# twice154/ofa-for-super-resolution

Hardware: AMD Instinct MI355X
Metric: sr_training_images_per_sec_4x_64to256 (higher is better)
Workload: dtype bf16; 1 GPU; OFA-SR S4 supernet 4x progressive shrinking (elastic kernel {3,5,7}, e=6, d=4, pd=2), LR 64x64 -> HR 256x256, fwd+bwd+Adam, train-mode BN; kernel_transform_mode=1, compat_reference_indexing=True, parallelism=dp1, per_gpu_batch=16, global_batch=16, grad_allreduce_bytes=0, launch=eager

## Files before the change

ofa-for-super-resolution_amd/csrc/pwconv.hip:

```cpp
#include <stdlib.h>
#include "ofasr_common.h"

namespace ofasr {

typedef __attribute__((ext_vector_type(16))) float f32x16;
typedef __attribute__((ext_vector_type(8))) __bf16 bf16x8;
typedef __attribute__((ext_vector_type(8))) _Float16 f16x8;
typedef __attribute__((ext_vector_type(4))) short s16x4;
typedef __attribute__((ext_vector_type(8))) short s16x8;
typedef __attribute__((address_space(3))) s16x4 lds_s16x4;

constexpr int PW_THREADS = 256;
constexpr int PW_TILE = 128;
constexpr int XROW16 = 320;
constexpr int XROW32 = 512;
constexpr int WROW16 = 128;
constexpr int WROW32 = 256;

template <typename T> struct Mma16;
template <> struct Mma16<bf16_t> {
    static __device__ __forceinline__ f32x16 run(s16x8 a, s16x8 b, f32x16 c) {
        return __builtin_amdgcn_mfma_f32_32x32x16_bf16(__builtin_bit_cast(bf16x8, a), __builtin_bit_cast(bf16x8, b),
                                                       c, 0, 0, 0);
    }
// ... 1177 lines not shown

template <typename T> struct Rows64 {
    static constexpr int NIT = Elem<T>::is16 ? 2 : 4;
    static constexpr int CPR = Elem<T>::is16 ? 8 : 16;
    static constexpr int EPC = Elem<T>::is16 ? 8 : 4;
    uint4 v[NIT];
    uint32_t ok;
};
template <typename T>
__device__ __forceinline__ void rows64_request(Rows64<T>& g, const T* __restrict__ base, int rows_total, int r0, int HW, int p0) {
    const int tid = threadIdx.x;
    g.ok = 0;
#pragma unroll
    for (int it = 0; it < Rows64<T>::NIT; ++it) {
        const int q = tid + it * PW_THREADS;
        const int r = q / Rows64<T>::CPR, ch = q % Rows64<T>::CPR;
        const int px = p0 + Rows64<T>::EPC * ch;
        const bool ok = r0 + r < rows_total && px < HW;
        g.v[it] = *reinterpret_cast<const uint4*>(base + (ok ? (long long)(r0 + r) * HW + px : 0));
        g.ok |= (ok ? 1u : 0u) << it;
    }
}
template <typename T>
__device__ __forceinline__ void rows64_deposit(char* Lt, const Rows64<T>& g) {
    const int tid = threadIdx.x;
#pragma unroll
    for (int it = 0; it < Rows64<T>::NIT; ++it) {
        const int q = tid + it * PW_THREADS;
        const int r = q / Rows64<T>::CPR, ch = q % Rows64<T>::CPR;
        const uint32_t m = (g.ok >> it) & 1u ? 0xffffffffu : 0u;
        *reinterpret_cast<uint4*>(Lt + wtile_chunk_off<T>(r, ch)) = make_uint4(g.v[it].x & m, g.v[it].y & m, g.v[it].z & m, g.v[it].w & m);
    }
}

template <typename T, bool ALIGNED>
__global__ void __launch_bounds__(PW_THREADS) pw_wgrad_kernel(const T* __restrict__ R, const T* __restrict__ S,
                                                              float* __restrict__ part, int MR, int NS, int HW,
                                                              int stages_per_img, int total_stages,
                                                              int stages_per_split) {
    constexpr int SUB = WgStage<T>::SUB;
    constexpr int TB = 64 * Elem<T>::wrow;
    __shared__ __attribute__((aligned(16))) char Rt[SUB * TB];
    __shared__ __attribute__((aligned(16))) char St[SUB * TB];
    const int r0 = blockIdx.x * 64, s0 = blockIdx.y * 64, z = blockIdx.z;
    const int lane = lane_id();
    const int wave = __builtin_amdgcn_readfirstlane((int)(threadIdx.x >> 6));
    const int c = lane & 31, h = lane >> 5;
    const int rb = wave & 1, sb = wave >> 1;
    f32x16 acc = zero16();
    const int q_lo = z * stages_per_split;
    const int q_hi = min(total_stages, q_lo + stages_per_split);
    auto multiply = [&]() {
#pragma unroll
        for (int sub = 0; sub < SUB; ++sub) {
            const char* Rs = Rt + sub * TB;
            const char* Ss = St + sub * TB;
            if constexpr (Elem<T>::is16) {
#pragma unroll
                for (int s = 0; s < 4; ++s) {
                    const s16x8 af = *reinterpret_cast<const s16x8*>(Rs + wtile_chunk_off<T>(32 * rb + c, 2 * s + h));
                    const s16x8 bf = *reinterpret_cast<const s16x8*>(Ss + wtile_chunk_off<T>(32 * sb + c, 2 * s + h));
                    acc = Mma16<T>::run(af, bf, acc);
                }
            } else {
#pragma unroll
                for (int s4 = 0; s4 < 8; ++s4) {
                    const float4 a4 = *reinterpret_cast<const float4*>(Rs + wtile_chunk_off<T>(32 * rb + c, 8 * h + s4));
                    const float4 b4 = *reinterpret_cast<const float4*>(Ss + wtile_chunk_off<T>(32 * sb + c, 8 * h + s4));
                    acc = __builtin_amdgcn_mfma_f32_32x32x2f32(a4.x, b4.x, acc, 0, 0, 0);
                    acc = __builtin_amdgcn_mfma_f32_32x32x2f32(a4.y, b4.y, acc, 0, 0, 0);
                    acc = __builtin_amdgcn_mfma_f32_32x32x2f32(a4.z, b4.z, acc, 0, 0, 0);
                    acc = __builtin_amdgcn_mfma_f32_32x32x2f32(a4.w, b4.w, acc, 0, 0, 0);
                }
            }
        }
    };
    if constexpr (ALIGNED) {
        Rows64<T> rg[SUB], sg[SUB];
        auto request = [&](int q) {
            const int n = q / stages_per_img;
            const int p0 = (q - n * stages_per_img) * (64 * SUB);
#pragma unroll
            for (int sub = 0; sub < SUB; ++sub) {
                rows64_request<T>(rg[sub], R + (long long)n * MR * HW, MR, r0, HW, p0 + 64 * sub);
                rows64_request<T>(sg[sub], S + (long long)n * NS * HW, NS, s0, HW, p0 + 64 * sub);
            }
        };
        if (q_lo < q_hi) request(q_lo);
        for (int q = q_lo; q < q_hi; ++q) {
            if (q > q_lo) __syncthreads();
#pragma unroll
            for (int sub = 0; sub < SUB; ++sub) {
                rows64_deposit<T>(Rt + sub * TB, rg[sub]);
                rows64_deposit<T>(St + sub * TB, sg[sub]);
            }
            __syncthreads();
            if (q + 1 < q_hi) request(q + 1);
            multiply();
        }
    } else {
        for (int q = q_lo; q < q_hi; ++q) {
            const int n = q / stages_per_img;
            const int p0 = (q - n * stages_per_img) * (64 * SUB);
            if (q > q_lo) __syncthreads();
#pragma unroll
            for (int sub = 0; sub < SUB; ++sub) {
                stage_rows64<T, ALIGNED>(Rt + sub * TB, R + (long long)n * MR * HW, MR, r0, HW, p0 + 64 * sub);
                stage_rows64<T, ALIGNED>(St + sub * TB, S + (long long)n * NS * HW, NS, s0, HW, p0 + 64 * sub);
            }
            __syncthreads();
            multiply();
        }
    }
    float* pz = part + (long long)z * MR * NS;
    const int sc = s0 + 32 * sb + c;
#pragma unroll
    for (int reg = 0; reg < 16; ++reg) {
        const int rr = r0 + 32 * rb + acc_row(reg, h);
        if (rr < MR && sc < NS) pz[(long long)rr * NS + sc] = acc[reg];
    }
}

constexpr int WR_ZL = 16;
__global__ void __launch_bounds__(64 * WR_ZL) pw_wgrad_reduce_kernel(const float* __restrict__ part,
                                                                     float* __restrict__ dw, int MR, int NS, int nsplit,
                                                                     long long sr, long long ss) {
    __shared__ float red[WR_ZL][64];
    const long long tot = (long long)MR * NS;
    const long long idx = (long long)blockIdx.x * 64 + (threadIdx.x & 63);
    const int zl = threadIdx.x >> 6;
    float a = 0.f;
    if (idx < tot) {
        int z = zl;
        for (; z + 3 * WR_ZL < nsplit; z += 4 * WR_ZL) {
            const float v0 = part[(long long)z * tot + idx], v1 = part[(long long)(z + WR_ZL) * tot + idx];
            const float v2 = part[(long long)(z + 2 * WR_ZL) * tot + idx], v3 = part[(long long)(z + 3 * WR_ZL) * tot + idx];
            a += (v0 + v1) + (v2 + v3);
        }
        for (; z < nsplit; z += WR_ZL) a += part[(long long)z * tot + idx];
    }
    red[zl][threadIdx.x & 63] = a;
    __syncthreads();
    if (zl == 0 && idx < tot) {
        float t = 0.f;
#pragma unroll
        for (int i = 0; i < WR_ZL; ++i) t += red[i][threadIdx.x];
        const long long r = idx / NS, sx = idx - r * NS;
        dw[r * sr + sx * ss] = t;
    }
}

constexpr int WD_RB = 3;
constexpr int WD_ROWS = 4 * WD_RB * 32, WD_COLS = 64;

struct WdPlan {
    int quads_per_img, total_quads, nsplit, MR, NS;
};

template <typename T, int XF = 0>
__global__ void __launch_bounds__(512) pw_wgrad_direct_kernel(const T* __restrict__ R, const T* __restrict__ S,
                                                              float* __restrict__ part, int MR, int NS, int HW,
                                                              WdPlan wp, InputXf xf = InputXf{}, BwdXf bx = BwdXf{}) {
    const int lane = lane_id();
    const int wave = __builtin_amdgcn_readfirstlane((int)(threadIdx.x >> 6));
    const int wr = wave & 3, wc = wave >> 2;
    const int c = lane & 31, h = lane >> 5;
    const int split = blockIdx.x;
    const int row0 = blockIdx.y * WD_ROWS + wr * (WD_RB * 32);
    const int col = blockIdx.z * WD_COLS + wc * 32 + c;
    if (row0 >= MR) return;
    f32x16 acc[WD_RB];
#pragma unroll
    for (int rb = 0; rb < WD_RB; ++rb) acc[rb] = zero16();
    const int q0 = (int)((long long)split * wp.total_quads / wp.nsplit);
    const int q1 = (int)((long long)(split + 1) * wp.total_quads / wp.nsplit);
    const bool cs = col < NS;
    const int colc = cs ? col : NS - 1;
    bool rs[WD_RB];
    int rowc[WD_RB];
#pragma unroll
    for (int rb = 0; rb < WD_RB; ++rb) {
        rs[rb] = row0 + 32 * rb + c < MR;
        rowc[rb] = rs[rb] ? row0 + 32 * rb + c : MR - 1;
    }
    float xsc[WD_RB], xmu[WD_RB], xb[WD_RB];
    float csc = 1.f, cmu = 0.f, cbb = 0.f;
    if constexpr (XF == 1) {
#pragma unroll
        for (int rb = 0; rb < WD_RB; ++rb) {
            xsc[rb] = xf.scale[rowc[rb]];
            xmu[rb] = xf.mean[rowc[rb]];
            xb[rb] = fmaf(xmu[rb], xsc[rb], xf.shift[rowc[rb]]);
        }
    }
    if constexpr (XF == 2) {
        csc = xf.scale[colc];
        cmu = xf.mean[colc];
        cbb = fmaf(cmu, csc, xf.shift[colc]);
    }
    float bka[WD_RB], bkbi[WD_RB];
    if constexpr (XF == 3) {
#pragma unroll
        for (int rb = 0; rb < WD_RB; ++rb) {
            xsc[rb] = bx.scale[rowc[rb]];
            xmu[rb] = bx.mean[rowc[rb]];
            xb[rb] = fmaf(xmu[rb], xsc[rb], bx.shift[rowc[rb]]);
            bka[rb] = bx.ka[rowc[rb]];
            bkbi[rb] = bx.kbi[rowc[rb]];
        }
    }
    long long rowoff[WD_RB];
#pragma unroll
    for (int rb = 0; rb < WD_RB; ++rb) rowoff[rb] = (long long)rowc[rb] * HW;
    const long long coloff = (long long)colc * HW;
    for (int q = q0; q < q1; ++q) {
        const int n = q / wp.quads_per_img;
        const int px = (q - n * wp.quads_per_img) * 64 + 32 * h;
        uint4 a[WD_RB][4], b[4];
        bool okp[4];
        int pxc[4];
#pragma unroll
        for (int j = 0; j < 4; ++j) {
            okp[j] = px + 8 * j < HW;
            pxc[j] = okp[j] ? px + 8 * j : 0;
        }
        const T* sp = S + (long long)n * NS * HW + coloff;
#pragma unroll
        for (int j = 0; j < 4; ++j) b[j] = *reinterpret_cast<const uint4*>(sp + pxc[j]);
        const T* rn = R + (long long)n * MR * HW;
#pragma unroll
        for (int rb = 0; rb < WD_RB; ++rb) {
#pragma unroll
            for (int j = 0; j < 4; ++j) {
                a[rb][j] = *reinterpret_cast<const uint4*>(rn + rowoff[rb] + pxc[j]);
            }
        }
        uint4 ya[XF == 3 ? WD_RB : 1][4];
        if constexpr (XF == 3) {
            const T* yn = reinterpret_cast<const T*>(bx.y) + (long long)n * MR * HW;
#pragma unroll
            for (int rb = 0; rb < WD_RB; ++rb) {
#pragma unroll
                for (int j = 0; j < 4; ++j)
                    ya[rb][j] = *reinterpret_cast<const uint4*>(yn + rowoff[rb] + pxc[j]);
            }
        }
#pragma unroll
        for (int j = 0; j < 4; ++j) {
            if constexpr (XF == 2) b[j] = xf_apply8_core<T>(b[j], csc, cmu, cbb);
            if (!(cs && okp[j])) b[j] = make_uint4(0, 0, 0, 0);
        }
#pragma unroll
        for (int rb = 0; rb < WD_RB; ++rb)
#pragma unroll
            for (int j = 0; j < 4; ++j) {
                if constexpr (XF == 1) a[rb][j] = xf_apply8_core<T>(a[rb][j], xsc[rb], xmu[rb], xb[rb]);
                if constexpr (XF == 3) a[rb][j] = bx_apply8<T>(a[rb][j], ya[rb][j], xmu[rb], xsc[rb], xb[rb], bka[rb], bkbi[rb]);
                if (!(rs[rb] && okp[j])) a[rb][j] = make_uint4(0, 0, 0, 0);
            }
#pragma unroll
        for (int j = 0; j < 4; ++j)
#pragma unroll
            for (int rb = 0; rb < WD_RB; ++rb)
                acc[rb] = Mma16<T>::run(__builtin_bit_cast(s16x8, a[rb][j]), __builtin_bit_cast(s16x8, b[j]), acc[rb]);
    }
    float* dst = part + (long long)split * MR * NS;
    if (cs) {
        float* p = dst + (long long)(row0 + 4 * h) * NS + col;
#pragma unroll
        for (int rb = 0; rb < WD_RB; ++rb)
#pragma unroll
            for (int reg = 0; reg < 16; ++reg) {
                const int r = row0 + 32 * rb + acc_row(reg, h);
                if (r < MR) *p = acc[rb][reg];
                p += (reg & 3) == 3 ? 5 * (long long)NS : (long long)NS;
            }
    }
}

static WdPlan wd_plan(int64_t N, int64_t Cin, int64_t Cout, int64_t HW) {
    WdPlan p;
    p.MR = (int)(Cout >= Cin ? Cout : Cin);
    p.NS = (int)(Cout >= Cin ? Cin : Cout);
    p.quads_per_img = (int)cdiv(HW, 64);
    p.total_quads = (int)(N * p.quads_per_img);
    const int64_t tiles = cdiv(p.MR, WD_ROWS) * cdiv(p.NS, WD_COLS);
    static const int blocks = [] { const char* e = getenv("OFASR_PW_WGRAD_BLOCKS"); const int v = e ? atoi(e) : 0; return v > 0 ? v : 256; }();
    int64_t want = blocks / (tiles > 0 ? tiles : 1);
    if (want > p.total_quads / 4) want = p.total_quads / 4;
    if (want < 1) want = 1;
    p.nsplit = (int)want;
    return p;
}


struct WdPlan32 {
    int units_per_img, total_units, nsplit, MR, NS;
};

__global__ void __launch_bounds__(512) pw_wgrad_direct_f32_kernel(const float* __restrict__ R, const float* __restrict__ S,
                                                                  float* __restrict__ part, int MR, int NS, int HW,
                                                                  WdPlan32 wp) {
    const int lane = lane_id();
    const int wave = __builtin_amdgcn_readfirstlane((int)(threadIdx.x >> 6));
    const int wr = wave & 3, wc = wave >> 2;
    const int c = lane & 31, h = lane >> 5;
    const int split = blockIdx.x;
    const int row0 = blockIdx.y * WD_ROWS + wr * (WD_RB * 32);
    const int col = blockIdx.z * WD_COLS + wc * 32 + c;
    if (row0 >= MR) return;
    f32x16 acc[WD_RB];
#pragma unroll
    for (int rb = 0; rb < WD_RB; ++rb) acc[rb] = zero16();
    const int u0 = (int)((long long)split * wp.total_units / wp.nsplit);
    const int u1 = (int)((long long)(split + 1) * wp.total_units / wp.nsplit);
    const bool cs = col < NS;
    const int colc = cs ? col : NS - 1;
    bool rs[WD_RB];
    long long rowoff[WD_RB];
#pragma unroll
    for (int rb = 0; rb < WD_RB; ++rb) {
        rs[rb] = row0 + 32 * rb + c < MR;
        rowoff[rb] = (long long)(rs[rb] ? row0 + 32 * rb + c : MR - 1) * HW;
    }
    float4 a[2][WD_RB][4], b[2][4];
    auto request = [&](int set, int u) {
        const int uc = u < u1 ? u : u1 - 1;
        const int n = uc / wp.units_per_img;
        const int px = (uc - n * wp.units_per_img) * 32 + 16 * h;
        int pxc[4];
#pragma unroll
        for (int j = 0; j < 4; ++j) pxc[j] = px + 4 * j < HW ? px + 4 * j : 0;
        const float* sp = S + ((long long)n * NS + colc) * HW;
        const float* rp = R + (long long)n * MR * HW;
#pragma unroll
        for (int j = 0; j < 4; ++j) b[set][j] = *reinterpret_cast<const float4*>(sp + pxc[j]);
#pragma unroll
        for (int rb = 0; rb < WD_RB; ++rb)
#pragma unroll
            for (int j = 0; j < 4; ++j) a[set][rb][j] = *reinterpret_cast<const float4*>(rp + rowoff[rb] + pxc[j]);
    };
    auto multiply = [&](int set, int u) {
        const int n = u / wp.units_per_img;
        const int px = (u - n * wp.units_per_img) * 32 + 16 * h;
        const bool live = u < u1;
#pragma unroll
        for (int j = 0; j < 4; ++j) {
            const bool ok = live && cs && px + 4 * j < HW;
            const float4 bv = ok ? b[set][j] : make_float4(0.f, 0.f, 0.f, 0.f);
#pragma unroll
            for (int rb = 0; rb < WD_RB; ++rb) {
                const float4 av = rs[rb] ? a[set][rb][j] : make_float4(0.f, 0.f, 0.f, 0.f);
                acc[rb] = __builtin_amdgcn_mfma_f32_32x32x2f32(av.x, bv.x, acc[rb], 0, 0, 0);
                acc[rb] = __builtin_amdgcn_mfma_f32_32x32x2f32(av.y, bv.y, acc[rb], 0, 0, 0);
                acc[rb] = __builtin_amdgcn_mfma_f32_32x32x2f32(av.z, bv.z, acc[rb], 0, 0, 0);
                acc[rb] = __builtin_amdgcn_mfma_f32_32x32x2f32(av.w, bv.w, acc[rb], 0, 0, 0);
            }
        }
    };
    if (u0 < u1) {
        request(0, u0);
        for (int u = u0; u < u1; u += 2) {
            request(1, u + 1);
            multiply(0, u);
            request(0, u + 2);
            multiply(1, u + 1);
        }
    }
    float* dst = part + (long long)split * MR * NS;
    if (cs) {
        float* p = dst + (long long)(row0 + 4 * h) * NS + col;
#pragma unroll
        for (int rb = 0; rb < WD_RB; ++rb)
#pragma unroll
            for (int reg = 0; reg < 16; ++reg) {
                const int r = row0 + 32 * rb + acc_row(reg, h);
                if (r < MR) *p = acc[rb][reg];
                p += (reg & 3) == 3 ? 5 * (long long)NS : (long long)NS;
            }
    }
}

static WdPlan32 wd_plan32(int64_t N, int64_t Cin, int64_t Cout, int64_t HW) {
    WdPlan32 p;
    p.MR = (int)(Cout >= Cin ? Cout : Cin);
    p.NS = (int)(Cout >= Cin ? Cin : Cout);
    p.units_per_img = (int)cdiv(HW, 32);
    p.total_units = (int)(N * p.units_per_img);
    const int64_t tiles = cdiv(p.MR, WD_ROWS) * cdiv(p.NS, WD_COLS);
    int64_t want = 256 / (tiles > 0 ? tiles : 1);
    if (want > p.total_units / 8) want = p.total_units / 8;
    if (want < 1) want = 1;
    p.nsplit = (int)want;
    return p;
}

struct WgradPlan {
    int stages_per_img, total_stages, nsplit, stages_per_split, MR, NS;
};

static WgradPlan wgrad_plan(int64_t N, int64_t Cin, int64_t Cout, int64_t HW, int sub) {
    WgradPlan p;
    p.MR = (int)(Cout >= Cin ? Cout : Cin);
    p.NS = (int)(Cout >= Cin ? Cin : Cout);
    p.stages_per_img = (int)cdiv(HW, 64 * sub);
    p.total_stages = (int)(N * p.stages_per_img);
    const int64_t tiles = cdiv(p.MR, 64) * cdiv(p.NS, 64);
    int64_t want = 512 / (tiles > 0 ? tiles : 1);
    if (want < 1) want = 1;
    if (want > p.total_stages) want = p.total_stages;
    if (want < 1) want = 1;
    p.stages_per_split = (int)cdiv(p.total_stages, want);
    if (p.stages_per_split < 1) p.stages_per_split = 1;
    p.nsplit = (int)cdiv(p.total_stages, p.stages_per_split);
    if (p.nsplit < 1) p.nsplit = 1;
    return p;
}

static bool aligned_for(const void* a, const void* b, int64_t HW, bool is16) {
    const uintptr_t bits = reinterpret_cast<uintptr_t>(a) | reinterpret_cast<uintptr_t>(b);
    return (bits & 15) == 0 && (HW % (is16 ? 8 : 4)) == 0;
}

template <typename T, bool AL, bool WV, bool XF = false>
static void launch_gemm_v(const void* x, WView wv, void* y, int64_t HW, int tiles_per_img, int total_tiles,
                          hipStream_t st, InputXf xf = InputXf{}, const void* addend = nullptr,
                          StatOut so = StatOut{nullptr, 0}, BnFold fold = BnFold{}) {
    if (wv.K <= 64) {
        if constexpr (Elem<T>::is16 && AL && WV && !XF) {
            static const bool slabs = [] { const char* e = getenv("OFASR_PW_FANOUT_SLABS"); return !(e && e[0] == '0'); }();
            const int nslab = wv.M / FO_ROWS;
            if (slabs && addend == nullptr && wv.K == 64 && wv.M % FO_ROWS == 0 && (nslab == 2 || nslab == 3) &&
                HW % PW_TILE == 0) {
                dim3 g1((unsigned)total_tiles);
#define OFASR_FO_SLABS(NS, ST)                                                                                       \
    OFASR_LAUNCH((pw_fanout_slabs_kernel<T, NS, ST>), g1, dim3(PW_THREADS), 0, st, (const T*)x, wv, (T*)y, (int)HW, \
                       tiles_per_img, so, BwdStatOut{})
                if (nslab == 3) { if (so.partial) OFASR_FO_SLABS(3, 1); else OFASR_FO_SLABS(3, 0); }
                else { if (so.partial) OFASR_FO_SLABS(2, 1); else OFASR_FO_SLABS(2, 0); }
#undef OFASR_FO_SLABS
                return;
            }
        }
        dim3 grid((unsigned)total_tiles, (unsigned)cdiv(wv.M, FO_ROWS));
        OFASR_LAUNCH((pw_fanout_kernel<T, AL, WV, XF>), grid, dim3(PW_THREADS), 0, st, (const T*)x, wv, (T*)y,
                           (int)HW, tiles_per_img, xf, (const T*)addend, so);
    } else {
        dim3 grid((unsigned)total_tiles, (unsigned)cdiv(wv.M, 64));
        if constexpr (Elem<T>::is16 && AL && WV) {
            static const bool fast_ok = [] { const char* e = getenv("OFASR_PW_FANIN_FAST"); return !(e && e[0] == '0'); }();
            const bool span32 = (long long)wv.K * HW < (1LL << 31) &&
                                (long long)wv.M * wv.sm + (long long)wv.K * wv.sk < (1LL << 31);
            if (fast_ok && wv.K % 4 == 0 && wv.M % 4 == 0 && span32)
                OFASR_LAUNCH((pw_fanin_pipe_kernel<T, XF, true>), grid, dim3(PW_THREADS), 0, st, (const T*)x, wv,
                                   (T*)y, (int)HW, tiles_per_img, (int)cdiv(wv.K, 64), xf, (const T*)addend, so, fold);
            else
                OFASR_LAUNCH((pw_fanin_pipe_kernel<T, XF, false>), grid, dim3(PW_THREADS), 0, st, (const T*)x, wv,
                                   (T*)y, (int)HW, tiles_per_img, (int)cdiv(wv.K, 64), xf, (const T*)addend, so, fold);
            return;
        }
        OFASR_LAUNCH((pw_fanin_kernel<T, AL, WV, XF>), grid, dim3(PW_THREADS), 0, st, (const T*)x, wv, (T*)y,
                           (int)HW, tiles_per_img, (int)cdiv(wv.K, 64), xf, (const T*)addend, so);
    }
}

template <typename T, bool XF = false>
static int launch_gemm(const char* name, const void* x, WView wv, void* y, int64_t N, int64_t HW, hipStream_t st,
                       InputXf xf = InputXf{}, const void* addend = nullptr, StatOut so = StatOut{nullptr, 0},
                       BnFold fold = BnFold{}) {
    constexpr bool is16 = Elem<T>::is16;
    const bool al = aligned_for(x, y, HW, is16);
    const long long ld = wv.sk == 1 ? wv.sm : wv.sk;
    const bool wvec = (reinterpret_cast<uintptr_t>(wv.w) & 15) == 0 && (ld % 4) == 0 && wv.K % 4 == 0 && wv.M % 4 == 0;
    const int tiles_per_img = (int)cdiv(HW, PW_TILE);
    const int64_t total64 = N * tiles_per_img;
    OFASR_REQUIRE(total64 <= INT32_MAX, OFASR_ERR_UNSUPPORTED, "%s: too many pixel tiles", name);
    const int total_tiles = (int)total64;
    {
        const double px = (double)N * (double)HW, es = (double)sizeof(T);
        prof_note(es * px * (wv.K + wv.M + (addend ? wv.M : 0)) + 4.0 * wv.K * wv.M, 2.0 * px * wv.K * wv.M);
    }
    if (so.partial)
        OFASR_REQUIRE(so.P == (wv.K <= 64 ? total_tiles : 2 * total_tiles), OFASR_ERR_INVALID_ARG,
                      "%s: statistics unit count %d does not match the launch", name, so.P);
    if constexpr (XF) {
        OFASR_REQUIRE(al && is16, OFASR_ERR_UNSUPPORTED, "%s: fused input transform needs aligned 16-bit tensors", name);
        if (fold.cp)
            OFASR_REQUIRE(wvec && wv.K > 64 && wv.K <= FOLD_KMAX, OFASR_ERR_UNSUPPORTED,
                          "%s: folded statistics need the pipelined fan-in kernel (64 < K <= %d)", name, FOLD_KMAX);
        if (wvec) launch_gemm_v<T, true, true, true>(x, wv, y, HW, tiles_per_img, total_tiles, st, xf, nullptr, so, fold);
        else launch_gemm_v<T, true, false, true>(x, wv, y, HW, tiles_per_img, total_tiles, st, xf, nullptr, so);
        return check_launch(name);
    }
    const bool al2 = al && (addend == nullptr || (reinterpret_cast<uintptr_t>(addend) & 15) == 0);
    if (al2 && wvec) launch_gemm_v<T, true, true>(x, wv, y, HW, tiles_per_img, total_tiles, st, InputXf{}, addend, so);
    else if (al2) launch_gemm_v<T, true, false>(x, wv, y, HW, tiles_per_img, total_tiles, st, InputXf{}, addend, so);
    else if (wvec) launch_gemm_v<T, false, true>(x, wv, y, HW, tiles_per_img, total_tiles, st, InputXf{}, addend, so);
    else launch_gemm_v<T, false, false>(x, wv, y, HW, tiles_per_img, total_tiles, st, InputXf{}, addend, so);
    return check_launch(name);
}

static int gemm_entry(const char* name, const void* x, WView wv, void* y, int64_t N, int64_t HW, int dtype,
                      void* stream, const void* addend = nullptr, StatOut so = StatOut{nullptr, 0}) {
    hipStream_t st = as_stream(stream);
    switch (dtype) {
        case OFASR_F32: return launch_gemm<float>(name, x, wv, y, N, HW, st, InputXf{}, addend, so);
        case OFASR_F16: return launch_gemm<f16_t>(name, x, wv, y, N, HW, st, InputXf{}, addend, so);
        default: return launch_gemm<bf16_t>(name, x, wv, y, N, HW, st, InputXf{}, addend, so);
    }
}

static int check_pw_args(const char* name, const void* a, const void* b, const void* c, int64_t ldw, int64_t N,
                         int64_t Cin, int64_t Cout, int64_t HW, int dtype) {
    OFASR_REQUIRE(a && b && c, OFASR_ERR_INVALID_ARG, "%s: null pointer", name);
    OFASR_REQUIRE(N >= 0 && Cin > 0 && Cout > 0 && HW >= 0, OFASR_ERR_INVALID_ARG,
                  "%s: bad shape N=%lld Cin=%lld Cout=%lld HW=%lld", name, (long long)N, (long long)Cin,
                  (long long)Cout, (long long)HW);
    OFASR_REQUIRE(ldw >= Cin, OFASR_ERR_INVALID_ARG, "%s: ldw=%lld < Cin=%lld", name, (long long)ldw, (long long)Cin);
    OFASR_REQUIRE(dtype == OFASR_F32 || dtype == OFASR_F16 || dtype == OFASR_BF16, OFASR_ERR_INVALID_ARG,
                  "%s: bad dtype %d", name, dtype);
    OFASR_REQUIRE(Cin <= 65536 && Cout <= 65536 && HW <= (1 << 30) && N <= (1 << 24), OFASR_ERR_UNSUPPORTED,
                  "%s: dimension too large", name);
    return OFASR_OK;
}

template <typename T, bool XF = false, bool BXM = false>
static int launch_wgrad(const char* name, const void* dy, const void* x, float* dw, int64_t ldw, int64_t N, int64_t Cin,
                        int64_t Cout, int64_t HW, float* ws, hipStream_t st, InputXf xf = InputXf{}, BwdXf bx = BwdXf{}) {
    const WgradPlan p = wgrad_plan(N, Cin, Cout, HW, WgStage<T>::SUB);
    const bool big_is_dy = Cout >= Cin;
    const T* R = (const T*)(big_is_dy ? dy : x);
    const T* S = (const T*)(big_is_dy ? x : dy);
    const long long sr = big_is_dy ? ldw : 1, ss = big_is_dy ? 1 : ldw;
    const bool al = aligned_for(dy, x, HW, Elem<T>::is16);
    prof_note((double)sizeof(T) * (double)N * (double)HW * (double)(Cin + Cout) + 4.0 * (double)Cin * (double)Cout,
              2.0 * (double)N * (double)HW * (double)Cin * (double)Cout);
    if constexpr (Elem<T>::is16) {
        if (al) {
            const WdPlan wp = wd_plan(N, Cin, Cout, HW);
            dim3 grid((unsigned)wp.nsplit, (unsigned)cdiv(wp.MR, WD_ROWS), (unsigned)cdiv(wp.NS, WD_COLS));
            if constexpr (XF) {
                if (big_is_dy)
                    OFASR_LAUNCH((pw_wgrad_direct_kernel<T, 2>), grid, dim3(512), 0, st, R, S, ws, wp.MR, wp.NS,
                                       (int)HW, wp, xf);
                else
                    OFASR_LAUNCH((pw_wgrad_direct_kernel<T, 1>), grid, dim3(512), 0, st, R, S, ws, wp.MR, wp.NS,
                                       (int)HW, wp, xf);
            } else if constexpr (BXM) {
                if (!big_is_dy) {
                    set_error("%s: the fused BN backward is implemented for the wide gradient operand (Cout >= Cin)", name);
                    return OFASR_ERR_UNSUPPORTED;
                }
                OFASR_LAUNCH((pw_wgrad_direct_kernel<T, 3>), grid, dim3(512), 0, st, R, S, ws, wp.MR, wp.NS, (int)HW, wp,
                             InputXf{}, bx);
            } else {
                OFASR_LAUNCH((pw_wgrad_direct_kernel<T>), grid, dim3(512), 0, st, R, S, ws, wp.MR, wp.NS, (int)HW,
                                   wp);
            }
            int rc = check_launch(name);
            if (rc) return rc;
            const long long tot = (long long)wp.MR * wp.NS;
            OFASR_LAUNCH(pw_wgrad_reduce_kernel, dim3((unsigned)cdiv(tot, 64)), dim3(64 * WR_ZL), 0, st, ws, dw, wp.MR,
                               wp.NS, wp.nsplit, sr, ss);
            return check_launch(name);
        }
    }
    if constexpr (XF || BXM) {
        set_error("%s: fused input transform needs the aligned 16-bit kernel", name);
        return OFASR_ERR_UNSUPPORTED;
    }
    if constexpr (!Elem<T>::is16) {
        static const bool f32_direct = [] { const char* e = getenv("OFASR_PW_WGRAD_F32_DIRECT"); return e && e[0] == '1'; }();
        if (al && f32_direct) {
            const WdPlan32 wp = wd_plan32(N, Cin, Cout, HW);
            dim3 grid((unsigned)wp.nsplit, (unsigned)cdiv(wp.MR, WD_ROWS), (unsigned)cdiv(wp.NS, WD_COLS));
            OFASR_LAUNCH(pw_wgrad_direct_f32_kernel, grid, dim3(512), 0, st, (const float*)R, (const float*)S, ws, wp.MR, wp.NS,
                         (int)HW, wp);
            int rc = check_launch(name);
            if (rc) return rc;
            const long long tot = (long long)wp.MR * wp.NS;
            OFASR_LAUNCH(pw_wgrad_reduce_kernel, dim3((unsigned)cdiv(tot, 64)), dim3(64 * WR_ZL), 0, st, ws, dw, wp.MR, wp.NS,
                         wp.nsplit, sr, ss);
            return check_launch(name);
        }
    }
    dim3 grid((unsigned)cdiv(p.MR, 64), (unsigned)cdiv(p.NS, 64), (unsigned)p.nsplit);
    if (al)
        OFASR_LAUNCH((pw_wgrad_kernel<T, true>), grid, dim3(PW_THREADS), 0, st, R, S, ws, p.MR, p.NS, (int)HW,
                           p.stages_per_img, p.total_stages, p.stages_per_split);
    else
        OFASR_LAUNCH((pw_wgrad_kernel<T, false>), grid, dim3(PW_THREADS), 0, st, R, S, ws, p.MR, p.NS, (int)HW,
                           p.stages_per_img, p.total_stages, p.stages_per_split);
    int rc = check_launch(name);
    if (rc) return rc;
    const long long tot = (long long)p.MR * p.NS;
    OFASR_LAUNCH(pw_wgrad_reduce_kernel, dim3((unsigned)cdiv(tot, 64)), dim3(64 * WR_ZL), 0, st, ws, dw, p.MR, p.NS,
                       p.nsplit, sr, ss);
    return check_launch(name);
}

int pwconv_dgrad_add(const void* dy, const float* w, int64_t ldw, void* dx, const void* addend, int64_t N, int64_t Cin,
                     int64_t Cout, int64_t HW, int dtype, void* stream) {
    const char* name = "pwconv_dgrad_add";
    int rc = check_pw_args(name, dy, w, dx, ldw, N, Cin, Cout, HW, dtype);
    if (rc) return rc;
    OFASR_REQUIRE(addend != nullptr, OFASR_ERR_INVALID_ARG, "%s: null addend", name);
    if (N * HW == 0) return OFASR_OK;
    WView wv{w, 1, ldw, (int)Cin, (int)Cout};
    return gemm_entry(name, dy, wv, dx, N, HW, dtype, stream, addend);
}

bool pwconv_dgrad_bx_supported(const void* da, const void* y, const void* dx, const void* addend, const float* w,
                               int64_t ldw, int64_t Cin, int64_t Cout, int64_t HW, int dtype) {
    if (dtype != OFASR_F16 && dtype != OFASR_BF16) return false;
    const uintptr_t bits = reinterpret_cast<uintptr_t>(da) | reinterpret_cast<uintptr_t>(y) | reinterpret_cast<uintptr_t>(dx) |
                           reinterpret_cast<uintptr_t>(addend) | reinterpret_cast<uintptr_t>(w);
    static const bool fast_ok = [] { const char* e = getenv("OFASR_PW_FANIN_FAST"); return !(e && e[0] == '0'); }();
    return fast_ok && (bits & 15) == 0 && HW % 8 == 0 && ldw % 4 == 0 && Cin % 4 == 0 && Cout % 4 == 0 && Cout > 64 &&
           Cout <= FOLD_KMAX && Cout * HW < (1LL << 31) && (Cin + Cout) * ldw < (1LL << 31);
}

template <typename T>
static int launch_dgrad_bx(const char* name, const void* da, WView wv, void* dx, const void* addend, int64_t N, int64_t HW,
                           BwdXf bx, hipStream_t st) {
    const int tiles_per_img = (int)cdiv(HW, PW_TILE);
    const int64_t total64 = N * tiles_per_img;
    OFASR_REQUIRE(total64 <= INT32_MAX, OFASR_ERR_UNSUPPORTED, "%s: too many pixel tiles", name);
    {
        const double px = (double)N * (double)HW, es = (double)sizeof(T);
        prof_note(es * px * (2.0 * wv.K + wv.M + (addend ? wv.M : 0)) + 4.0 * wv.K * wv.M, 2.0 * px * wv.K * wv.M);
    }
    dim3 grid((unsigned)total64, (unsigned)cdiv(wv.M, 64));
    OFASR_LAUNCH((pw_fanin_pipe_kernel<T, false, true, true>), grid, dim3(PW_THREADS), 0, st, (const T*)da, wv, (T*)dx,
                 (int)HW, tiles_per_img, (int)cdiv(wv.K, 64), InputXf{}, (const T*)addend, StatOut{nullptr, 0}, BnFold{}, bx);
    return check_launch(name);
}

int pwconv_dgrad_add_bx(const void* da, const float* w, int64_t ldw, void* dx, const void* addend, int64_t N, int64_t Cin,
                        int64_t Cout, int64_t HW, int dtype, BwdXf bx, void* stream) {
    const char* name = "pwconv_dgrad_add_bx";
    int rc = check_pw_args(name, da, w, dx, ldw, N, Cin, Cout, HW, dtype);
    if (rc) return rc;
    OFASR_REQUIRE(bx.y && bx.mean && bx.scale && bx.shift &&
                      ((bx.ka && bx.kbi) || (bx.fold_partial && bx.fold_invstd && bx.fold_P > 0 && bx.fold_C == Cout)),
                  OFASR_ERR_INVALID_ARG, "%s: null transform", name);
    OFASR_REQUIRE(pwconv_dgrad_bx_supported(da, bx.y, dx, addend, w, ldw, Cin, Cout, HW, dtype), OFASR_ERR_UNSUPPORTED,
                  "%s: needs the pipelined fan-in kernel (aligned 16-bit tensors, 64 < Cout <= %d)", name, FOLD_KMAX);
    if (N * HW == 0) return OFASR_OK;
    WView wv{w, 1, ldw, (int)Cin, (int)Cout};
    hipStream_t st = as_stream(stream);
    if (dtype == OFASR_F16) return launch_dgrad_bx<f16_t>(name, da, wv, dx, addend, N, HW, bx, st);
    return launch_dgrad_bx<bf16_t>(name, da, wv, dx, addend, N, HW, bx, st);
}

bool pwconv_xf_supported(const void* x, const void* y, int64_t HW, int dtype) {
    return (dtype == OFASR_F16 || dtype == OFASR_BF16) && aligned_for(x, y, HW, true);
}

bool pwconv_dgrad_bstat_supported(const void* dy, const void* y, const void* dx, const float* w, int64_t ldw, int64_t Cin,
                                  int64_t Cout, int64_t HW, int dtype) {
    const bool wvec = (reinterpret_cast<uintptr_t>(w) & 15) == 0 && (ldw % 4) == 0;
    return (dtype == OFASR_F16 || dtype == OFASR_BF16) && aligned_for(dy, dx, HW, true) &&
           (reinterpret_cast<uintptr_t>(y) & 15) == 0 && wvec && Cout == 64 && (Cin == 2 * FO_ROWS || Cin == 3 * FO_ROWS) &&
           HW % PW_TILE == 0;
}

template <typename T>
static int launch_dgrad_bstat(const void* dy, WView wv, void* dx, int64_t N, int64_t HW, BwdStatOut bs, hipStream_t st) {
    const int tiles_per_img = (int)(HW / PW_TILE);
    const int total_tiles = (int)(N * tiles_per_img);
    const double px = (double)N * (double)HW;
    prof_note(2.0 * px * (wv.K + 2.0 * wv.M) + 4.0 * wv.K * wv.M, 2.0 * px * wv.K * wv.M);
    if (wv.M == 3 * FO_ROWS)
        OFASR_LAUNCH((pw_fanout_slabs_kernel<T, 3, 2>), dim3((unsigned)total_tiles), dim3(PW_THREADS), 0, st, (const T*)dy, wv,
                     (T*)dx, (int)HW, tiles_per_img, StatOut{nullptr, 0}, bs);
    else
        OFASR_LAUNCH((pw_fanout_slabs_kernel<T, 2, 2>), dim3((unsigned)total_tiles), dim3(PW_THREADS), 0, st, (const T*)dy, wv,
                     (T*)dx, (int)HW, tiles_per_img, StatOut{nullptr, 0}, bs);
    return check_launch("pwconv_dgrad_bstat");
}

int pwconv_dgrad_bstat(const void* dy, const float* w, int64_t ldw, void* dx, int64_t N, int64_t Cin, int64_t Cout,
                       int64_t HW, int dtype, BwdStatOut bs, void* stream) {
    const char* name = "pwconv_dgrad_bstat";
    int rc = check_pw_args(name, dy, w, dx, ldw, N, Cin, Cout, HW, dtype);
    if (rc) return rc;
    OFASR_REQUIRE(bs.y && bs.mean && bs.scale && bs.shift && bs.partial, OFASR_ERR_INVALID_ARG, "%s: null pointer", name);
    OFASR_REQUIRE(pwconv_dgrad_bstat_supported(dy, bs.y, dx, w, ldw, Cin, Cout, HW, dtype), OFASR_ERR_UNSUPPORTED,
                  "%s: shape outside the slab-walk kernel", name);
    OFASR_REQUIRE(N * (HW / PW_TILE) <= INT32_MAX && bs.P == (int)(N * (HW / PW_TILE)), OFASR_ERR_INVALID_ARG,
                  "%s: unit count %d does not match the launch", name, bs.P);
    WView wv{w, 1, ldw, (int)Cin, (int)Cout};
    hipStream_t st = as_stream(stream);
    if (dtype == OFASR_F16) return launch_dgrad_bstat<f16_t>(dy, wv, dx, N, HW, bs, st);
    return launch_dgrad_bstat<bf16_t>(dy, wv, dx, N, HW, bs, st);
}

int pwconv_stat_units(int64_t N, int64_t Cin, int64_t HW) {
    const int64_t tiles = N * cdiv(HW, PW_TILE);
    return (int)(Cin <= 64 ? tiles : 2 * tiles);
}

int pwconv_fwd_stat(const void* x, const float* w, int64_t ldw, void* y, int64_t N, int64_t Cin, int64_t Cout,
                    int64_t HW, int dtype, StatOut so, void* stream) {
    const char* name = "pwconv_fwd_stat";
    int rc = check_pw_args(name, x, w, y, ldw, N, Cin, Cout, HW, dtype);
    if (rc) return rc;
    OFASR_REQUIRE(so.partial != nullptr && N * HW > 0, OFASR_ERR_INVALID_ARG, "%s: null statistics / empty tensor", name);
    WView wv{w, ldw, 1, (int)Cout, (int)Cin};
    return gemm_entry(name, x, wv, y, N, HW, dtype, stream, nullptr, so);
}

bool pwconv_fold_supported(const void* x, const void* y, const float* w, int64_t ldw, int64_t Cin, int64_t HW, int dtype) {
    const bool wvec = (reinterpret_cast<uintptr_t>(w) & 15) == 0 && (ldw % 4) == 0;
    return pwconv_xf_supported(x, y, HW, dtype) && wvec && Cin > 64 && Cin <= FOLD_KMAX && Cin % 4 == 0;
}

int pwconv_fwd_fold(const void* x, const float* w, int64_t ldw, void* y, int64_t N, int64_t Cin, int64_t Cout,
                    int64_t HW, int dtype, BnFold fold, void* stream, StatOut so) {
    const char* name = "pwconv_fwd_fold";
    int rc = check_pw_args(name, x, w, y, ldw, N, Cin, Cout, HW, dtype);
    if (rc) return rc;
    OFASR_REQUIRE(fold.cp && fold.P > 0 && fold.mean && fold.invstd && fold.scale && fold.shift, OFASR_ERR_INVALID_ARG,
                  "%s: incomplete statistics source", name);
    OFASR_REQUIRE(dtype == OFASR_F16 || dtype == OFASR_BF16, OFASR_ERR_UNSUPPORTED, "%s: 16-bit only", name);
    OFASR_REQUIRE(N * HW > 0, OFASR_ERR_UNSUPPORTED, "%s: empty tensor", name);
    WView wv{w, ldw, 1, (int)Cout, (int)Cin};
    hipStream_t st = as_stream(stream);
    if (dtype == OFASR_F16) return launch_gemm<f16_t, true>(name, x, wv, y, N, HW, st, InputXf{}, nullptr, so, fold);
    return launch_gemm<bf16_t, true>(name, x, wv, y, N, HW, st, InputXf{}, nullptr, so, fold);
}

int pwconv_fwd_xf(const void* x, const float* w, int64_t ldw, void* y, int64_t N, int64_t Cin, int64_t Cout, int64_t HW,
                  int dtype, InputXf xf, void* stream, StatOut so) {
    const char* name = "pwconv_fwd_xf";
    int rc = check_pw_args(name, x, w, y, ldw, N, Cin, Cout, HW, dtype);
    if (rc) return rc;
    OFASR_REQUIRE(xf.scale && xf.shift && xf.mean, OFASR_ERR_INVALID_ARG, "%s: null transform", name);
    OFASR_REQUIRE(dtype == OFASR_F16 || dtype == OFASR_BF16, OFASR_ERR_UNSUPPORTED, "%s: 16-bit only", name);
    if (N * HW == 0) return OFASR_OK;
    WView wv{w, ldw, 1, (int)Cout, (int)Cin};
    hipStream_t st = as_stream(stream);
    if (dtype == OFASR_F16) return launch_gemm<f16_t, true>(name, x, wv, y, N, HW, st, xf, nullptr, so);
    return launch_gemm<bf16_t, true>(name, x, wv, y, N, HW, st, xf, nullptr, so);
}

int pwconv_wgrad_xf(const void* dy, const void* x, float* dw, int64_t ldw, int64_t N, int64_t Cin, int64_t Cout,
                    int64_t HW, int dtype, InputXf xf, void* workspace, size_t workspace_bytes, void* stream) {
    const char* name = "pwconv_wgrad_xf";
    int rc = check_pw_args(name, dy, x, dw, ldw, N, Cin, Cout, HW, dtype);
    if (rc) return rc;
    OFASR_REQUIRE(xf.scale && xf.shift && xf.mean, OFASR_ERR_INVALID_ARG, "%s: null transform", name);
    OFASR_REQUIRE(dtype == OFASR_F16 || dtype == OFASR_BF16, OFASR_ERR_UNSUPPORTED, "%s: 16-bit only", name);
    OFASR_REQUIRE(N * HW > 0, OFASR_ERR_UNSUPPORTED, "%s: empty tensor", name);
    const size_t need = ofasr_pwconv_wgrad_workspace(N, Cin, Cout, HW);
    OFASR_REQUIRE(workspace && workspace_bytes >= need, OFASR_ERR_WORKSPACE, "%s: workspace %zu B < required %zu B",
                  name, workspace_bytes, need);
    hipStream_t st = as_stream(stream);
    if (dtype == OFASR_F16)
        return launch_wgrad<f16_t, true>(name, dy, x, dw, ldw, N, Cin, Cout, HW, (float*)workspace, st, xf);
    return launch_wgrad<bf16_t, true>(name, dy, x, dw, ldw, N, Cin, Cout, HW, (float*)workspace, st, xf);
}

bool pwconv_wgrad_bx_supported(const void* da, const void* y, const void* x, int64_t Cin, int64_t Cout, int64_t HW, int dtype) {
    if (!(dtype == OFASR_F16 || dtype == OFASR_BF16) || Cout < Cin) return false;
    return aligned_for(da, x, HW, true) && aligned_for(y, x, HW, true);
}

int pwconv_wgrad_bx(const void* da, const void* x, float* dw, int64_t ldw, int64_t N, int64_t Cin, int64_t Cout, int64_t HW,
                    int dtype, BwdXf bx, void* workspace, size_t workspace_bytes, void* stream) {
    const char* name = "pwconv_wgrad_bx";
    int rc = check_pw_args(name, da, x, dw, ldw, N, Cin, Cout, HW, dtype);
    if (rc) return rc;
    OFASR_REQUIRE(bx.y && bx.mean && bx.scale && bx.shift && bx.ka && bx.kbi, OFASR_ERR_INVALID_ARG, "%s: null transform", name);
    OFASR_REQUIRE(pwconv_wgrad_bx_supported(da, bx.y, x, Cin, Cout, HW, dtype), OFASR_ERR_UNSUPPORTED,
                  "%s: needs 16-bit aligned tensors and Cout >= Cin", name);
    OFASR_REQUIRE(N * HW > 0, OFASR_ERR_UNSUPPORTED, "%s: empty tensor", name);
    const size_t need = ofasr_pwconv_wgrad_workspace(N, Cin, Cout, HW);
    OFASR_REQUIRE(workspace && workspace_bytes >= need, OFASR_ERR_WORKSPACE, "%s: workspace %zu B < required %zu B",
                  name, workspace_bytes, need);
    hipStream_t st = as_stream(stream);
    if (dtype == OFASR_F16)
        return launch_wgrad<f16_t, false, true>(name, da, x, dw, ldw, N, Cin, Cout, HW, (float*)workspace, st, InputXf{}, bx);
    return launch_wgrad<bf16_t, false, true>(name, da, x, dw, ldw, N, Cin, Cout, HW, (float*)workspace, st, InputXf{}, bx);
}

}

using namespace ofasr;

OFASR_EXPORT int ofasr_pwconv_fwd(const void* x, const float* w, int64_t ldw, void* y, int64_t N, int64_t Cin,
                                  int64_t Cout, int64_t HW, int dtype, void* stream) {
    const char* name = "ofasr_pwconv_fwd";
    int rc = check_pw_args(name, x, w, y, ldw, N, Cin, Cout, HW, dtype);
    if (rc) return rc;
    if (N * HW == 0) return OFASR_OK;
    WView wv{w, ldw, 1, (int)Cout, (int)Cin};
    return gemm_entry(name, x, wv, y, N, HW, dtype, stream);
}

OFASR_EXPORT int ofasr_pwconv_dgrad(const void* dy, const float* w, int64_t ldw, void* dx, int64_t N, int64_t Cin,
                                    int64_t Cout, int64_t HW, int dtype, void* stream) {
    const char* name = "ofasr_pwconv_dgrad";
    int rc = check_pw_args(name, dy, w, dx, ldw, N, Cin, Cout, HW, dtype);
    if (rc) return rc;
    if (N * HW == 0) return OFASR_OK;
    WView wv{w, 1, ldw, (int)Cin, (int)Cout};
    return gemm_entry(name, dy, wv, dx, N, HW, dtype, stream);
}

OFASR_EXPORT size_t ofasr_pwconv_wgrad_workspace(int64_t N, int64_t Cin, int64_t Cout, int64_t HW) {
    if (N <= 0 || Cin <= 0 || Cout <= 0 || HW <= 0) return 0;
    const WgradPlan p4 = wgrad_plan(N, Cin, Cout, HW, 4), p2 = wgrad_plan(N, Cin, Cout, HW, 2);
    int ns = p4.nsplit > p2.nsplit ? p4.nsplit : p2.nsplit;
    const int nd = wd_plan(N, Cin, Cout, HW).nsplit;
    ns = nd > ns ? nd : ns;
    const int nd32 = wd_plan32(N, Cin, Cout, HW).nsplit;
    ns = nd32 > ns ? nd32 : ns;
    return (size_t)ns * (size_t)p4.MR * (size_t)p4.NS * sizeof(float);
}

OFASR_EXPORT int ofasr_pwconv_wgrad(const void* dy, const void* x, float* dw, int64_t ldw, int64_t N, int64_t Cin,
                                    int64_t Cout, int64_t HW, int dtype, void* workspace, size_t workspace_bytes,
                                    void* stream) {
    const char* name = "ofasr_pwconv_wgrad";
    int rc = check_pw_args(name, dy, x, dw, ldw, N, Cin, Cout, HW, dtype);
    if (rc) return rc;
    hipStream_t st = as_stream(stream);
    if (N * HW == 0) {
        for (int64_t co = 0; co < Cout; ++co) {
            hipError_t e = hipMemsetAsync(dw + co * ldw, 0, (size_t)Cin * sizeof(float), st);
            OFASR_REQUIRE(e == hipSuccess, OFASR_ERR_LAUNCH, "%s: memset failed", name);
        }
        return OFASR_OK;
    }
    const size_t need = ofasr_pwconv_wgrad_workspace(N, Cin, Cout, HW);
    OFASR_REQUIRE(workspace && workspace_bytes >= need, OFASR_ERR_WORKSPACE, "%s: workspace %zu B < required %zu B",
                  name, workspace_bytes, need);
    float* ws = (float*)workspace;
    switch (dtype) {
        case OFASR_F32: return launch_wgrad<float>(name, dy, x, dw, ldw, N, Cin, Cout, HW, ws, st);
        case OFASR_F16: return launch_wgrad<f16_t>(name, dy, x, dw, ldw, N, Cin, Cout, HW, ws, st);
        default: return launch_wgrad<bf16_t>(name, dy, x, dw, ldw, N, Cin, Cout, HW, ws, st);
    }
}
```

Baseline: 2712 images/s.

## Stage pointwise wgrad operands through double-buffered LDS with cooperative coalesced loads

The direct pointwise weight-gradient kernel previously had each wave load its own A and B fragments straight from global memory, so operands were re-fetched redundantly across waves. It now loads the 384-row by 64-column tile cooperatively with 16-byte chunks, applies the fused BN transforms once, writes into a double-buffered LDS stage, and has waves read MFMA fragments from LDS while the next quad is prefetched into registers. A row-count dispatch picks 3, 4 or 6 load iterations so partial row tiles do less work. The cost is extra LDS traffic, a barrier per quad, higher dynamic shared memory use per block and possible occupancy loss. Debug exports for the fused variants are also added.

```diff
diff --git a/ofa-for-super-resolution_amd/csrc/pwconv.hip b/ofa-for-super-resolution_amd/csrc/pwconv.hip
--- a/ofa-for-super-resolution_amd/csrc/pwconv.hip
+++ b/ofa-for-super-resolution_amd/csrc/pwconv.hip
@@ -1353,45 +1353,73 @@
 
 constexpr int WD_RB = 3;
 constexpr int WD_ROWS = 4 * WD_RB * 32, WD_COLS = 64;
+constexpr int WD_STAGE_BYTES = (WD_ROWS + WD_COLS) * WROW16;
+constexpr int WD_LDS_BYTES = 2 * WD_STAGE_BYTES;
 
 struct WdPlan {
     int quads_per_img, total_quads, nsplit, MR, NS;
 };
 
-template <typename T, int XF = 0>
-__global__ void __launch_bounds__(512) pw_wgrad_direct_kernel(const T* __restrict__ R, const T* __restrict__ S,
-                                                              float* __restrict__ part, int MR, int NS, int HW,
-                                                              WdPlan wp, InputXf xf = InputXf{}, BwdXf bx = BwdXf{}) {
+template <typename T, int XF, int NRIT>
+__device__ __forceinline__ void wd_body(char* smem, const T* __restrict__ R, const T* __restrict__ S,
+                                        float* __restrict__ part, int MR, int NS, int HW, const WdPlan& wp,
+                                        const InputXf& xf, const BwdXf& bx) {
+    constexpr int NBLK = 2 * NRIT;
+    constexpr int NRB = (NBLK + 3) / 4;
+    const int tid = threadIdx.x;
     const int lane = lane_id();
     const int wave = __builtin_amdgcn_readfirstlane((int)(threadIdx.x >> 6));
     const int wr = wave & 3, wc = wave >> 2;
     const int c = lane & 31, h = lane >> 5;
     const int split = blockIdx.x;
-    const int row0 = blockIdx.y * WD_ROWS + wr * (WD_RB * 32);
-    const int col = blockIdx.z * WD_COLS + wc * 32 + c;
-    if (row0 >= MR) return;
-    f32x16 acc[WD_RB];
-#pragma unroll
-    for (int rb = 0; rb < WD_RB; ++rb) acc[rb] = zero16();
+    const int rbase = blockIdx.y * WD_ROWS, cbase = blockIdx.z * WD_COLS;
     const int q0 = (int)((long long)split * wp.total_quads / wp.nsplit);
     const int q1 = (int)((long long)(split + 1) * wp.total_quads / wp.nsplit);
-    const bool cs = col < NS;
-    const int colc = cs ? col : NS - 1;
-    bool rs[WD_RB];
-    int rowc[WD_RB];
-#pragma unroll
-    for (int rb = 0; rb < WD_RB; ++rb) {
-        rs[rb] = row0 + 32 * rb + c < MR;
-        rowc[rb] = rs[rb] ? row0 + 32 * rb + c : MR - 1;
-    }
-    float xsc[WD_RB], xmu[WD_RB], xb[WD_RB];
+    const int ch = tid & 7, rg = tid >> 3;
+    bool rv[NRIT];
+    int rowc[NRIT];
+    long long roff[NRIT];
+#pragma unroll
+    for (int it = 0; it < NRIT; ++it) {
+        const int r = rbase + 64 * it + rg;
+        rv[it] = r < MR;
+        rowc[it] = rv[it] ? r : MR - 1;
+        roff[it] = (long long)rowc[it] * HW;
+    }
+    const bool sv = cbase + rg < NS;
+    const int colc = sv ? cbase + rg : NS - 1;
+    const long long soff = (long long)colc * HW;
+
+    uint4 a[NRIT], b, ya[XF == 3 ? NRIT : 1];
+    const T *rp, *sp, *yp;
+    auto address = [&](int q) -> bool {
+        const int n = q / wp.quads_per_img;
+        const int px = (q - n * wp.quads_per_img) * 64 + 8 * ch;
+        const bool ok = px < HW;
+        const int pxc = ok ? px : 0;
+        rp = R + (long long)n * MR * HW + pxc;
+        sp = S + (long long)n * NS * HW + soff + pxc;
+        if constexpr (XF == 3) yp = reinterpret_cast<const T*>(bx.y) + (long long)n * MR * HW + pxc;
+        return ok;
+    };
+    bool okp = false;
+    if (q0 < q1) {
+        okp = address(q0);
+#pragma unroll
+        for (int it = 0; it < NRIT; ++it) {
+            a[it] = *reinterpret_cast<const uint4*>(rp + roff[it]);
+            if constexpr (XF == 3) ya[it] = *reinterpret_cast<const uint4*>(yp + roff[it]);
+        }
+        b = *reinterpret_cast<const uint4*>(sp);
+    }
+    float xsc[NRIT], xmu[NRIT], xb[NRIT], bka[NRIT], bkbi[NRIT];
     float csc = 1.f, cmu = 0.f, cbb = 0.f;
     if constexpr (XF == 1) {
 #pragma unroll
-        for (int rb = 0; rb < WD_RB; ++rb) {
-            xsc[rb] = xf.scale[rowc[rb]];
-            xmu[rb] = xf.mean[rowc[rb]];
-            xb[rb] = fmaf(xmu[rb], xsc[rb], xf.shift[rowc[rb]]);
+        for (int it = 0; it < NRIT; ++it) {
+            xsc[it] = xf.scale[rowc[it]];
+            xmu[it] = xf.mean[rowc[it]];
+            xb[it] = fmaf(xmu[it], xsc[it], xf.shift[rowc[it]]);
         }
     }
     if constexpr (XF == 2) {
@@ -1399,84 +1427,102 @@
         cmu = xf.mean[colc];
         cbb = fmaf(cmu, csc, xf.shift[colc]);
     }
-    float bka[WD_RB], bkbi[WD_RB];
     if constexpr (XF == 3) {
 #pragma unroll
-        for (int rb = 0; rb < WD_RB; ++rb) {
-            xsc[rb] = bx.scale[rowc[rb]];
-            xmu[rb] = bx.mean[rowc[rb]];
-            xb[rb] = fmaf(xmu[rb], xsc[rb], bx.shift[rowc[rb]]);
-            bka[rb] = bx.ka[rowc[rb]];
-            bkbi[rb] = bx.kbi[rowc[rb]];
-        }
-    }
-    long long rowoff[WD_RB];
-#pragma unroll
-    for (int rb = 0; rb < WD_RB; ++rb) rowoff[rb] = (long long)rowc[rb] * HW;
-    const long long coloff = (long long)colc * HW;
+        for (int it = 0; it < NRIT; ++it) {
+            xsc[it] = bx.scale[rowc[it]];
+            xmu[it] = bx.mean[rowc[it]];
+            xb[it] = fmaf(xmu[it], xsc[it], bx.shift[rowc[it]]);
+            bka[it] = bx.ka[rowc[it]];
+            bkbi[it] = bx.kbi[rowc[it]];
+        }
+    }
+    const uint4 zero4 = make_uint4(0, 0, 0, 0);
+    auto deposit = [&](char* buf, int qn, auto more) {
+        constexpr bool MORE = decltype(more)::value;
+        const bool ok = okp;
+        if constexpr (MORE) okp = address(qn);
+#pragma unroll
+        for (int it = 0; it < NRIT; ++it) {
+            uint4 v = a[it];
+            if constexpr (XF == 1) v = xf_apply8_core<T>(v, xsc[it], xmu[it], xb[it]);
+            if constexpr (XF == 3) v = bx_apply8<T>(v, ya[it], xmu[it], xsc[it], xb[it], bka[it], bkbi[it]);
+            if (!(rv[it] && ok)) v = zero4;
+            *reinterpret_cast<uint4*>(buf + wtile_chunk_off<T>(64 * it + rg, ch)) = v;
+            if constexpr (MORE) {
+                a[it] = *reinterpret_cast<const uint4*>(rp + roff[it]);
+                if constexpr (XF == 3) ya[it] = *reinterpret_cast<const uint4*>(yp + roff[it]);
+            }
+        }
+        uint4 v = b;
+        if constexpr (XF == 2) v = xf_apply8_core<T>(v, csc, cmu, cbb);
+        if (!(sv && ok)) v = zero4;
+        *reinterpret_cast<uint4*>(buf + wtile_chunk_off<T>(WD_ROWS + rg, ch)) = v;
+        if constexpr (MORE) b = *reinterpret_cast<const uint4*>(sp);
+    };
+    f32x16 acc[WD_RB];
+#pragma unroll
+    for (int rb = 0; rb < WD_RB; ++rb) acc[rb] = zero16();
+    bool bv[NRB];
+    int arow[NRB];
+#pragma unroll
+    for (int rb = 0; rb < NRB; ++rb) {
+        bv[rb] = 4 * rb + wr < NBLK && rbase + 32 * (4 * rb + wr) < MR;
+        arow[rb] = 32 * (bv[rb] ? 4 * rb + wr : wr) + c;
+    }
+    auto multiply = [&](const char* buf) {
+#pragma unroll
+        for (int s = 0; s < 4; ++s) {
+            const s16x8 bf = *reinterpret_cast<const s16x8*>(buf + wtile_chunk_off<T>(WD_ROWS + 32 * wc + c, 4 * h + s));
+#pragma unroll
+            for (int rb = 0; rb < NRB; ++rb) {
+                const s16x8 af = *reinterpret_cast<const s16x8*>(buf + wtile_chunk_off<T>(arow[rb], 4 * h + s));
+                acc[rb] = Mma16<T>::run(af, bf, acc[rb]);
+            }
+        }
+    };
     for (int q = q0; q < q1; ++q) {
-        const int n = q / wp.quads_per_img;
-        const int px = (q - n * wp.quads_per_img) * 64 + 32 * h;
-        uint4 a[WD_RB][4], b[4];
-        bool okp[4];
-        int pxc[4];
-#pragma unroll
-        for (int j = 0; j < 4; ++j) {
-            okp[j] = px + 8 * j < HW;
-            pxc[j] = okp[j] ? px + 8 * j : 0;
-        }
-        const T* sp = S + (long long)n * NS * HW + coloff;
-#pragma unroll
-        for (int j = 0; j < 4; ++j) b[j] = *reinterpret_cast<const uint4*>(sp + pxc[j]);
-        const T* rn = R + (long long)n * MR * HW;
-#pragma unroll
-        for (int rb = 0; rb < WD_RB; ++rb) {
-#pragma unroll
-            for (int j = 0; j < 4; ++j) {
-                a[rb][j] = *reinterpret_cast<const uint4*>(rn + rowoff[rb] + pxc[j]);
-            }
-        }
-        uint4 ya[XF == 3 ? WD_RB : 1][4];
-        if constexpr (XF == 3) {
-            const T* yn = reinterpret_cast<const T*>(bx.y) + (long long)n * MR * HW;
-#pragma unroll
-            for (int rb = 0; rb < WD_RB; ++rb) {
-#pragma unroll
-                for (int j = 0; j < 4; ++j)
-                    ya[rb][j] = *reinterpret_cast<const uint4*>(yn + rowoff[rb] + pxc[j]);
-            }
-        }
-#pragma unroll
-        for (int j = 0; j < 4; ++j) {
-            if constexpr (XF == 2) b[j] = xf_apply8_core<T>(b[j], csc, cmu, cbb);
-            if (!(cs && okp[j])) b[j] = make_uint4(0, 0, 0, 0);
-        }
-#pragma unroll
-        for (int rb = 0; rb < WD_RB; ++rb)
-#pragma unroll
-            for (int j = 0; j < 4; ++j) {
-                if constexpr (XF == 1) a[rb][j] = xf_apply8_core<T>(a[rb][j], xsc[rb], xmu[rb], xb[rb]);
-                if constexpr (XF == 3) a[rb][j] = bx_apply8<T>(a[rb][j], ya[rb][j], xmu[rb], xsc[rb], xb[rb], bka[rb], bkbi[rb]);
-                if (!(rs[rb] && okp[j])) a[rb][j] = make_uint4(0, 0, 0, 0);
-            }
-#pragma unroll
-        for (int j = 0; j < 4; ++j)
-#pragma unroll
-            for (int rb = 0; rb < WD_RB; ++rb)
-                acc[rb] = Mma16<T>::run(__builtin_bit_cast(s16x8, a[rb][j]), __builtin_bit_cast(s16x8, b[j]), acc[rb]);
-    }
-    float* dst = part + (long long)split * MR * NS;
-    if (cs) {
-        float* p = dst + (long long)(row0 + 4 * h) * NS + col;
-#pragma unroll
-        for (int rb = 0; rb < WD_RB; ++rb)
+        char* buf = smem + ((q - q0) & 1) * WD_STAGE_BYTES;
+        if (q + 1 < q1) deposit(buf, q + 1, std::true_type{});
+        else deposit(buf, q, std::false_type{});
+        lds_barrier();
+        multiply(buf);
+    }
+    const int col = cbase + 32 * wc + c;
+    if (col < NS) {
+        float* dst = part + (long long)split * MR * NS + col;
+#pragma unroll
+        for (int rb = 0; rb < NRB; ++rb) {
+            if (!bv[rb]) continue;
+            const int row0 = rbase + 32 * (4 * rb + wr);
+            float* p = dst + (long long)(row0 + 4 * h) * NS;
 #pragma unroll
             for (int reg = 0; reg < 16; ++reg) {
-                const int r = row0 + 32 * rb + acc_row(reg, h);
-                if (r < MR) *p = acc[rb][reg];
+                if (row0 + acc_row(reg, h) < MR) *p = acc[rb][reg];
                 p += (reg & 3) == 3 ? 5 * (long long)NS : (long long)NS;
             }
-    }
+        }
+    }
+}
+
+template <typename T, int XF = 0>
+__global__ void __launch_bounds__(512) pw_wgrad_direct_kernel(const T* __restrict__ R, const T* __restrict__ S,
+                                                              float* __restrict__ part, int MR, int NS, int HW,
+                                                              WdPlan wp, InputXf xf = InputXf{}, BwdXf bx = BwdXf{}) {
+    extern __shared__ __attribute__((aligned(16))) char wd_smem[];
+    const int rows = MR - (int)blockIdx.y * WD_ROWS;
+    if (rows > 256) wd_body<T, XF, 6>(wd_smem, R, S, part, MR, NS, HW, wp, xf, bx);
+    else if (rows > 192) wd_body<T, XF, 4>(wd_smem, R, S, part, MR, NS, HW, wp, xf, bx);
+    else wd_body<T, XF, 3>(wd_smem, R, S, part, MR, NS, HW, wp, xf, bx);
+}
+
+template <typename T, int XF>
+static void wd_launch(dim3 grid, hipStream_t st, const T* R, const T* S, float* ws, int HW, const WdPlan& wp,
+                      InputXf xf = InputXf{}, BwdXf bx = BwdXf{}) {
+    static const bool attr = ((void)hipFuncSetAttribute(reinterpret_cast<const void*>(&pw_wgrad_direct_kernel<T, XF>),
+                                                        hipFuncAttributeMaxDynamicSharedMemorySize, WD_LDS_BYTES), true);
+    (void)attr;
+    OFASR_LAUNCH((pw_wgrad_direct_kernel<T, XF>), grid, dim3(512), WD_LDS_BYTES, st, R, S, ws, wp.MR, wp.NS, HW, wp, xf, bx);
 }
 
 static WdPlan wd_plan(int64_t N, int64_t Cin, int64_t Cout, int64_t HW) {
@@ -1741,22 +1787,16 @@
             const WdPlan wp = wd_plan(N, Cin, Cout, HW);
             dim3 grid((unsigned)wp.nsplit, (unsigned)cdiv(wp.MR, WD_ROWS), (unsigned)cdiv(wp.NS, WD_COLS));
             if constexpr (XF) {
-                if (big_is_dy)
-                    OFASR_LAUNCH((pw_wgrad_direct_kernel<T, 2>), grid, dim3(512), 0, st, R, S, ws, wp.MR, wp.NS,
-                                       (int)HW, wp, xf);
-                else
-                    OFASR_LAUNCH((pw_wgrad_direct_kernel<T, 1>), grid, dim3(512), 0, st, R, S, ws, wp.MR, wp.NS,
-                                       (int)HW, wp, xf);
+                if (big_is_dy) wd_launch<T, 2>(grid, st, R, S, ws, (int)HW, wp, xf);
+                else wd_launch<T, 1>(grid, st, R, S, ws, (int)HW, wp, xf);
             } else if constexpr (BXM) {
                 if (!big_is_dy) {
                     set_error("%s: the fused BN backward is implemented for the wide gradient operand (Cout >= Cin)", name);
                     return OFASR_ERR_UNSUPPORTED;
                 }
-                OFASR_LAUNCH((pw_wgrad_direct_kernel<T, 3>), grid, dim3(512), 0, st, R, S, ws, wp.MR, wp.NS, (int)HW, wp,
-                             InputXf{}, bx);
+                wd_launch<T, 3>(grid, st, R, S, ws, (int)HW, wp, InputXf{}, bx);
             } else {
-                OFASR_LAUNCH((pw_wgrad_direct_kernel<T>), grid, dim3(512), 0, st, R, S, ws, wp.MR, wp.NS, (int)HW,
-                                   wp);
+                wd_launch<T, 0>(grid, st, R, S, ws, (int)HW, wp);
             }
             int rc = check_launch(name);
             if (rc) return rc;
@@ -2045,3 +2085,25 @@
         default: return launch_wgrad<bf16_t>(name, dy, x, dw, ldw, N, Cin, Cout, HW, ws, st);
     }
 }
+
+
+OFASR_EXPORT int ofasr_debug_pwconv_wgrad_xf(const void* dy, const void* x, float* dw, int64_t ldw, int64_t N, int64_t Cin,
+                                             int64_t Cout, int64_t HW, int dtype, const float* scale, const float* shift,
+                                             const float* mean, void* workspace, size_t workspace_bytes, void* stream) {
+    return pwconv_wgrad_xf(dy, x, dw, ldw, N, Cin, Cout, HW, dtype, InputXf{scale, shift, mean}, workspace, workspace_bytes,
+                           stream);
+}
+
+OFASR_EXPORT int ofasr_debug_pwconv_wgrad_bx(const void* da, const void* y, const void* x, float* dw, int64_t ldw, int64_t N,
+                                             int64_t Cin, int64_t Cout, int64_t HW, int dtype, const float* mean,
+                                             const float* scale, const float* shift, const float* ka, const float* kbi,
+                                             void* workspace, size_t workspace_bytes, void* stream) {
+    BwdXf bx{};
+    bx.y = y;
+    bx.mean = mean;
+    bx.scale = scale;
+    bx.shift = shift;
+    bx.ka = ka;
+    bx.kbi = kbi;
+    return pwconv_wgrad_bx(da, x, dw, ldw, N, Cin, Cout, HW, dtype, bx, workspace, workspace_bytes, stream);
+}
```

Result: faster. 2773 images/s, median of 6 (+2.3%).
